# browserdotsys/vecchio

Hardware: NVIDIA B200
Metric: Mpaths/s (higher is better)
Workload: dtype f32

## Files before the change

vecchio_b200/csrc/vk_warpq.cu:

```cuda
#include "vk_warpq.cuh"

namespace VK_NS {

template <bool MEDIA, bool LEGACY, class W, int K, bool HYBRID, class D>
VKD void warpq_flat_body(const DScene& sc, const FlatProgram* flat, const DCamera& cam, const RenderArgs& a, const RenderBuffers& buf,
                         unsigned long long* unit_head, const D& dom) {
    extern __shared__ __align__(16) unsigned char vkq_raw[];
    const uint32_t lane = threadIdx.x & 31u, below = (1u << lane) - 1u;
    W& S = reinterpret_cast<W*>(vkq_raw)[threadIdx.x >> 5];
    const WqCtx<W> C = wq_ctx(dom, cam, a, S, unit_head, lane);
    uint32_t n_rays = 0, n_drop = 0, n_prims = 0;
    TraceCounters tc = {0u, 0u};
    constexpr uint32_t EXT_CAP = 32u * K;
    const uint32_t miss_cls = wq_black_miss(a) ? (uint32_t)VKQ_END : (uint32_t)VKQ_EMIT;
    wq_init(S, lane);
#pragma unroll 1
    for (;;) {
        uint32_t q, n_q, tail_q, head;
        wq_selfcheck(S, buf, lane, 0u);
        if (!wq_pick(S, wq_counts(S), EXT_CAP, q, n_q, tail_q)) break;
        const uint32_t n = wq_pop(S, q, n_q, tail_q, q == VKQ_EXT ? EXT_CAP : 32u, lane, head);
        if (q != VKQ_EXT) {
            wq_shade_batch<LEGACY, !HYBRID>(sc, C, dom, buf, q, n, head, n_drop);
            continue;
        }
        wq_converge();
        float3 o[K], d[K];
        float tm[K], best_t[K];
        bool live[K];
        uint32_t best_hit[K], slot[K];
        MediumXi xi[K];
#pragma unroll
        for (int k = 0; k < K; ++k) {
            const uint32_t e = lane + 32u * k;
            live[k] = e < n;
            slot[k] = S.ring[VKQ_EXT][(head + (live[k] ? e : 0u)) & W::RMASK];
            const float4 ro = S.ro[slot[k]], rd = S.rd[slot[k]];
            o[k] = f3(ro);
            d[k] = f3(rd);
            tm[k] = ro.w;
            xi[k].table = nullptr;
            xi[k].depth = __float_as_uint(rd.w);
            xi[k].rng.key = make_uint2(a.seed_lo, a.seed_hi);
            xi[k].rng.pixel = MEDIA ? S.px[slot[k]] : 0u;
            xi[k].rng.sample = MEDIA ? __float_as_uint(S.bt[slot[k]].w) : 0u;
            if (MEDIA) dom_slot_rng(dom, a, xi[k].rng);
        }
        TraceHit sub[K];
        trace_flat_k<K, MEDIA, HYBRID>(sc, *flat, o, d, tm, live, 0.001f, xi, best_t, best_hit, sub, &tc);
#pragma unroll
        for (int k = 0; k < K; ++k) {
            uint32_t cls = VKQ_NONE;
            if (live[k]) {
                ++n_rays;
                n_prims += flat->n;
                uint32_t prim = VK_REF_NONE, hi = 0u;
                cls = miss_cls;
                if (HYBRID && best_hit[k] == 0xFFFFFFFEu) {
                    prim = sub[k].prim;
                    hi = (sub[k].inst ? (0x80000000u | VKD_INDEX(sub[k].inst)) : 0u) | (sub[k].face << 28);
                    cls = wq_class_of(sc, prim, sub[k].inst);
                } else if (best_hit[k] != 0xFFFFFFFFu) {
                    cls = best_hit[k] >> 8;
                    best_hit[k] = VKF_HIT_INDEX(best_hit[k]);
                    prim = 1u;
                    if (HYBRID) {
                        const FlatHit& fh = flat->hits[best_hit[k]];
                        prim = fh.prim & ~VKD_DUP;
                        hi = (fh.inst ? (0x80000000u | VKD_INDEX(fh.inst)) : 0u) | (fh.face << 28);
                    }
                }
                S.hp[slot[k]] = make_uint4(__float_as_uint(best_t[k]), prim, hi, best_hit[k]);
            }
            if (k == 0 || n > 32u * k) wq_push(S, cls, slot[k], lane, below);
        }
    }
    wq_flush_counters(buf, lane, n_rays, n_drop, tc.nodes, n_prims + tc.prims);
}

#ifndef VKQ_BVH_IDLE
#define VKQ_BVH_IDLE 8u
#endif
#ifndef VKQ_NODE_STEPS
#define VKQ_NODE_STEPS 4
#endif
template <bool MEDIA, bool LEGACY, class W, class D>
VKD void warpq_bvh_body(const DScene& sc, const DCamera& cam, const RenderArgs& a, const RenderBuffers& buf, unsigned long long* unit_head,
                        const D& dom) {
    extern __shared__ __align__(16) unsigned char vkq_raw[];
    const uint32_t lane = threadIdx.x & 31u, below = (1u << lane) - 1u;
    W& S = reinterpret_cast<W*>(vkq_raw)[threadIdx.x >> 5];
    const WqCtx<W> C = wq_ctx(dom, cam, a, S, unit_head, lane);
    uint32_t n_rays = 0, n_drop = 0;
    TraceCounters tc = {0u, 0u};
    const uint32_t miss_cls = wq_black_miss(a) ? (uint32_t)VKQ_END : (uint32_t)VKQ_EMIT;
    wq_init(S, lane);

    Trav T;
    T.ref = VKD_DONE;
    T.sp = 0;
    T.enter = false;
    T.cur_inst = 0;
    T.co = T.cd = T.cinv = f3(0.0f, 0.0f, 0.0f);
    T.best.t = 0.0f;
    T.best.prim = VK_REF_NONE;
    T.best.inst = 0;
    T.best.face = 0;
    float3 o = f3(0.0f, 0.0f, 0.0f), d = o;
    float tm = 0.0f;
    uint32_t cur = 0xFFFFFFFFu;
    MediumXi xi;
    xi.table = nullptr;
    xi.depth = 0;
    xi.rng.key = make_uint2(a.seed_lo, a.seed_hi);
    xi.rng.pixel = 0;
    xi.rng.sample = 0;
#pragma unroll 1
    for (;;) {
        const bool done_lane = T.ref == VKD_DONE;
        const uint32_t m_done = __ballot_sync(0xFFFFFFFFu, done_lane);
        if ((uint32_t)__popc(m_done) >= VKQ_BVH_IDLE) {
            const bool fin = done_lane && cur != 0xFFFFFFFFu;
            if (__ballot_sync(0xFFFFFFFFu, fin) != 0u) {
                uint32_t cls = VKQ_NONE, slot = 0u;
                if (fin) {
                    slot = cur;
                    cur = 0xFFFFFFFFu;
                    S.hp[slot] = make_uint4(__float_as_uint(T.best.t), T.best.prim,
                                            (T.best.inst ? (0x80000000u | VKD_INDEX(T.best.inst)) : 0u) | (T.best.face << 28), 0u);
                    cls = T.best.prim == VK_REF_NONE ? miss_cls : wq_class_of(sc, T.best.prim, T.best.inst);
                }
                wq_push(S, cls, slot, lane, below);
            }
            wq_selfcheck(S, buf, lane, (uint32_t)__popc(__ballot_sync(0xFFFFFFFFu, cur != 0xFFFFFFFFu)));
            const WqCounts cnt = wq_counts(S);
            const uint32_t n_ext = __reduce_max_sync(0xFFFFFFFFu, cnt.c01.x);
            if (n_ext != 0u) {
                uint32_t head;
                const uint32_t take = wq_pop(S, VKQ_EXT, n_ext, cnt.c01.y, (uint32_t)__popc(m_done), lane, head);
                const uint32_t rank = (uint32_t)__popc(m_done & below);
                if (done_lane && rank < take) {
                    cur = S.ring[VKQ_EXT][(head + rank) & W::RMASK];
                    const float4 ro = S.ro[cur], rd = S.rd[cur];
                    o = f3(ro);
                    d = f3(rd);
                    tm = ro.w;
                    xi.depth = __float_as_uint(rd.w);
                    if (MEDIA) {
                        xi.rng.pixel = S.px[cur];
                        xi.rng.sample = __float_as_uint(S.bt[cur].w);
                        dom_slot_rng(dom, a, xi.rng);
                    }
                    trav_init(T, sc, o, d, CUDART_INF_F);
                    ++n_rays;
                }
            }
            const uint32_t m_act = __ballot_sync(0xFFFFFFFFu, T.ref != VKD_DONE);
            if (32u - (uint32_t)__popc(m_act) >= VKQ_BVH_IDLE) {
                uint32_t q, n_q, tail_q, head;
                if (wq_pick(S, wq_counts(S), 0u, q, n_q, tail_q)) {
                    const uint32_t n = wq_pop(S, q, n_q, tail_q, 32u, lane, head);
                    wq_shade_batch<LEGACY, false>(sc, C, dom, buf, q, n, head, n_drop);
                    continue;
                }
                if (m_act == 0u) break;
            }
        }
        wq_converge();
#pragma unroll 1
        for (int k = 0; k < VKQ_NODE_STEPS && trav_at_node(T); ++k) trav_node_step(T, sc, 0.001f, tc);
        if (T.ref != VKD_DONE && !trav_at_node(T)) trav_prim_step<MEDIA>(T, sc, o, d, tm, 0.001f, xi, tc);
    }
    wq_flush_counters(buf, lane, n_rays, n_drop, tc.nodes, tc.prims);
}

using WqFlat = WqWarp<VKQ_N_FLAT, VKQ_RN_FLAT>;
using WqMedia = WqWarp<VKQ_N_MEDIA, VKQ_RN_MEDIA>;
using WqBvh = WqWarp<VKQ_N_BVH, VKQ_RN_BVH>;
using WqHyb = WqWarp<VKQ_N_HYB, VKQ_RN_HYB>;
static_assert(VKQ_WARPS <= 15, "one named barrier per warp of the CTA");

template <bool MEDIA, bool LEGACY, class D>
__global__ void __launch_bounds__(32 * VKQ_WARPS, VKQ_MINB_BVH) k_warpq(const DScene sc, const DCamera cam, const RenderArgs a, const RenderBuffers buf,
                                                                    unsigned long long* unit_head, const __grid_constant__ D dom) {
    warpq_bvh_body<MEDIA, LEGACY, WqBvh>(sc, cam, a, buf, unit_head, dom);
}
template <bool LEGACY, class D>
__global__ void __launch_bounds__(32 * VKQ_WARPS, VKQ_MINB_FLAT) k_warpq_flat(const DScene sc, const __grid_constant__ FlatProgram flat, const DCamera cam,
                                                                          const RenderArgs a, const RenderBuffers buf, unsigned long long* unit_head,
                                                                          const __grid_constant__ D dom) {
    warpq_flat_body<false, LEGACY, WqFlat, VKQ_K_FLAT, false>(sc, &flat, cam, a, buf, unit_head, dom);
}
template <bool LEGACY, class D>
__global__ void __launch_bounds__(32 * VKQ_WARPS, VKQ_MINB_MEDIA) k_warpq_flat_media(const DScene sc, const __grid_constant__ FlatProgram flat,
                                                                                 const DCamera cam, const RenderArgs a, const RenderBuffers buf,
                                                                                 unsigned long long* unit_head, const __grid_constant__ D dom) {
    warpq_flat_body<true, LEGACY, WqMedia, VKQ_K_MEDIA, false>(sc, &flat, cam, a, buf, unit_head, dom);
}
#if !VK_SIMPLE
template <bool MEDIA, bool LEGACY, class D>
__global__ void __launch_bounds__(32 * VKQ_WARPS, VKQ_MINB_HYB) k_warpq_hybrid(const DScene sc, const __grid_constant__ FlatProgram flat, const DCamera cam,
                                                                            const RenderArgs a, const RenderBuffers buf, unsigned long long* unit_head,
                                                                            const __grid_constant__ D dom) {
    warpq_flat_body<MEDIA, LEGACY, WqHyb, 1, true>(sc, &flat, cam, a, buf, unit_head, dom);
}
#endif

template <class D>
cudaError_t launch_warpq(const DScene& sc, const FlatProgram* flat, const DCamera& cam, const RenderArgs& a, const RenderBuffers& b,
                         unsigned long long* unit_head, int sm_count, bool legacy, cudaStream_t st, const D& dom) {
    int bps = 0;
    cudaError_t e;
    const bool media = sc.has_media != 0u;
#define VKQ_LAUNCH_FLAT(KERNEL, WARP)                                                                                  \
    {                                                                                                                  \
        const size_t smem = VKQ_WARPS * sizeof(WARP);                                                                  \
        if ((e = warpq_prepare(KERNEL, smem, &bps)) != cudaSuccess) return e;                                          \
        KERNEL<<<sm_count * (bps < 1 ? 1 : bps), 32 * VKQ_WARPS, smem, st>>>(sc, *flat, cam, a, b, unit_head, dom);    \
    }
#define VKQ_LAUNCH_BVH(KERNEL)                                                                                         \
    {                                                                                                                  \
        const size_t smem = VKQ_WARPS * sizeof(WqBvh);                                                                 \
        if ((e = warpq_prepare(KERNEL, smem, &bps)) != cudaSuccess) return e;                                          \
        KERNEL<<<sm_count * (bps < 1 ? 1 : bps), 32 * VKQ_WARPS, smem, st>>>(sc, cam, a, b, unit_head, dom);           \
    }
#if VK_SIMPLE
    (void)legacy;
    if (media) VKQ_LAUNCH_FLAT((k_warpq_flat_media<false, D>), WqMedia) else VKQ_LAUNCH_FLAT((k_warpq_flat<false, D>), WqFlat)
#else
#define VKQ_LAUNCH_HYB(M, G) VKQ_LAUNCH_FLAT((k_warpq_hybrid<M, G, D>), WqHyb)
    if (flat && flat->n && flat->n_bvh) {
        if (media) { if (legacy) VKQ_LAUNCH_HYB(true, true) else VKQ_LAUNCH_HYB(true, false) }
        else { if (legacy) VKQ_LAUNCH_HYB(false, true) else VKQ_LAUNCH_HYB(false, false) }
    } else if (flat && flat->n) {
        if (media) { if (legacy) VKQ_LAUNCH_FLAT((k_warpq_flat_media<true, D>), WqMedia) else VKQ_LAUNCH_FLAT((k_warpq_flat_media<false, D>), WqMedia) }
        else { if (legacy) VKQ_LAUNCH_FLAT((k_warpq_flat<true, D>), WqFlat) else VKQ_LAUNCH_FLAT((k_warpq_flat<false, D>), WqFlat) }
    } else {
        if (media) { if (legacy) VKQ_LAUNCH_BVH((k_warpq<true, true, D>)) else VKQ_LAUNCH_BVH((k_warpq<true, false, D>)) }
        else { if (legacy) VKQ_LAUNCH_BVH((k_warpq<false, true, D>)) else VKQ_LAUNCH_BVH((k_warpq<false, false, D>)) }
    }
#undef VKQ_LAUNCH_HYB
#endif
#undef VKQ_LAUNCH_FLAT
#undef VKQ_LAUNCH_BVH
    return cudaGetLastError();
}
#define VKQ_INSTANTIATE(D)                                                                                             \
    template cudaError_t launch_warpq(const DScene&, const FlatProgram*, const DCamera&, const RenderArgs&, const RenderBuffers&, \
                                      unsigned long long*, int, bool, cudaStream_t, const D&);
VKQ_INSTANTIATE(OneFrame)
VKQ_INSTANTIATE(FrameArgs)
VKQ_INSTANTIATE(ListArgs)
VKQ_INSTANTIATE(FrameListArgs)
#undef VKQ_INSTANTIATE

}
```

vecchio_b200/csrc/vk_warpq.cuh:

```cuda
#pragma once
#include "vk_device.cuh"

namespace VK_NS {

#ifndef VKQ_WARPS
#define VKQ_WARPS 4
#endif
#ifndef VKQ_N_FLAT
#define VKQ_N_FLAT 176
#endif
#ifndef VKQ_RN_FLAT
#define VKQ_RN_FLAT 256
#endif
#ifndef VKQ_K_FLAT
#define VKQ_K_FLAT 2
#endif
#ifndef VKQ_MINB_FLAT
#define VKQ_MINB_FLAT 4
#endif
#ifndef VKQ_N_MEDIA
#define VKQ_N_MEDIA 144
#endif
#ifndef VKQ_RN_MEDIA
#define VKQ_RN_MEDIA 256
#endif
#ifndef VKQ_K_MEDIA
#define VKQ_K_MEDIA 1
#endif
#ifndef VKQ_MINB_MEDIA
#define VKQ_MINB_MEDIA 5
#endif
#ifndef VKQ_N_BVH
#define VKQ_N_BVH 120
#endif
#ifndef VKQ_RN_BVH
#define VKQ_RN_BVH 128
#endif
#ifndef VKQ_MINB_BVH
#define VKQ_MINB_BVH 6
#endif
#ifndef VKQ_N_HYB
#define VKQ_N_HYB 120
#endif
#ifndef VKQ_RN_HYB
#define VKQ_RN_HYB 128
#endif
#ifndef VKQ_MINB_HYB
#define VKQ_MINB_HYB 6
#endif
#ifndef VKQ_REGEN_MIN
#define VKQ_REGEN_MIN 32u
#endif
#define VKQ_CHUNK 256u
enum { VKQ_EXT = 0, VKQ_END = 1, VKQ_EMIT = 2, VKQ_DIEL = 3, VKQ_METAL = 4, VKQ_DIFF = 5, VKQ_DIFFI = 6, VKQ_NQ = 7,
       VKQ_SPH = 7, VKQ_BOX = 8, VKQ_LEAF = 9, VKQ_NQ_STEP = 10, VKQ_NONE = 15 };
static_assert(VKF_HITC(0, 0, 0) >> 8 == VKQ_EMIT && VKF_HITC(0, 1, 0) >> 8 == VKQ_DIEL && VKF_HITC(0, 2, 0) >> 8 == VKQ_METAL &&
              VKF_HITC(0, 3, 0) >> 8 == VKQ_DIFF && VKF_HITC(0, 3, 1) >> 8 == VKQ_DIFFI, "the flat program's class-tagged ids name these queues");

template <int N_, int RN_>
struct WqWarp {
    static constexpr uint32_t N = N_, RMASK = RN_ - 1, NQ = VKQ_NQ;
    static_assert((RN_ & (RN_ - 1)) == 0 && RN_ >= N_ && RN_ <= 256, "ring capacity: power of two, >= slots, byte indices");
    float4 ro[N_];
    float4 rd[N_];
    float4 bt[N_];
    uint4 hp[N_];
    uint32_t px[N_];
    uint8_t ring[VKQ_NQ][RN_];
    uint2 ct[8];
    uint32_t cur_s, cur_y, cur_x, left;
    uint32_t exhausted;
    VKD void mark_new(uint32_t) {}
};


#ifndef VKQ_CONVERGE
#define VKQ_CONVERGE 1
#endif
VKD void wq_converge() {
#if VKQ_CONVERGE
    asm volatile("barrier.sync.aligned %0, 32;" ::"r"((threadIdx.x >> 5) + 1u) : "memory");
#endif
}
template <class W>
struct WqCtx {
    const DCamera& cam;
    const RenderArgs& a;
    W& S;
    uint32_t chunks_per_row, chunks_per_sample;
    unsigned long long n_chunks;
    unsigned long long* unit_head;
    uint32_t lane, below;
};

template <class D> VKD uint32_t wq_row_length(const D&, const RenderArgs& a) { return a.width; }
VKD uint32_t wq_row_length(const ListArgs& ls, const RenderArgs&) { return ls.n; }
VKD uint32_t wq_row_length(const FrameListArgs& fl, const RenderArgs&) { return fl.ls.n; }
template <class D> VKD uint32_t wq_rows(const D&, const RenderArgs& a) { return a.height; }
VKD uint32_t wq_rows(const ListArgs&, const RenderArgs&) { return 1u; }
VKD uint32_t wq_rows(const FrameListArgs&, const RenderArgs&) { return 1u; }
template <class W, class D>
VKD WqCtx<W> wq_ctx(const D& dom, const DCamera& cam, const RenderArgs& a, W& S, unsigned long long* unit_head, uint32_t lane) {
    const uint32_t cpr = (wq_row_length(dom, a) + VKQ_CHUNK - 1u) / VKQ_CHUNK, cps = cpr * wq_rows(dom, a);
    return WqCtx<W>{cam, a, S, cpr, cps, (unsigned long long)cps * a.spp_count * dom_frames(dom), unit_head, lane, (1u << lane) - 1u};
}
template <class W>
VKD void wq_chunk(const WqCtx<W>& C, const OneFrame&, unsigned long long c) {
    W& S = C.S;
    const uint32_t sb = (uint32_t)(c / C.chunks_per_sample);
    const uint32_t r = (uint32_t)(c - (unsigned long long)sb * C.chunks_per_sample);
    const uint32_t row = r / C.chunks_per_row, x0 = (r - row * C.chunks_per_row) * VKQ_CHUNK;
    S.left = min(VKQ_CHUNK, C.a.width - x0);
    S.cur_s = sb;
    S.cur_y = row;
    S.cur_x = x0;
}
template <class W>
VKD void wq_chunk(const WqCtx<W>& C, const FrameArgs&, unsigned long long c) {
    W& S = C.S;
    const unsigned long long fs = c / C.chunks_per_sample;
    const uint32_t f = (uint32_t)(fs / C.a.spp_count);
    const uint32_t r = (uint32_t)(c - fs * C.chunks_per_sample);
    const uint32_t row = r / C.chunks_per_row, x0 = (r - row * C.chunks_per_row) * VKQ_CHUNK;
    S.left = min(VKQ_CHUNK, C.a.width - x0);
    S.cur_s = (uint32_t)(fs - (unsigned long long)f * C.a.spp_count);
    S.cur_y = f * C.a.height + row;
    S.cur_x = x0;
}
template <class W>
VKD void wq_chunk(const WqCtx<W>& C, const ListArgs& ls, unsigned long long c) {
    W& S = C.S;
    const uint32_t sb = (uint32_t)(c / C.chunks_per_sample);
    const uint32_t x0 = ((uint32_t)c - sb * C.chunks_per_sample) * VKQ_CHUNK;
    S.left = min(VKQ_CHUNK, ls.n - x0);
    S.cur_s = sb;
    S.cur_y = 0u;
    S.cur_x = x0;
}
template <class W>
VKD void wq_chunk(const WqCtx<W>& C, const FrameListArgs& fl, unsigned long long c) { wq_chunk(C, fl.ls, c); }
template <class W>
VKD uint32_t wq_camera_ray(const WqCtx<W>& C, const OneFrame&, uint32_t x, uint32_t y, PathRng& rng, float3& o, float3& d, float& time) {
    camera_get_ray(C.cam, rng, x, y, C.a.width, C.a.height, o, d, time);
    return rng.pixel;
}
template <class W>
VKD uint32_t wq_camera_ray(const WqCtx<W>& C, const FrameArgs& fr, uint32_t x, uint32_t y, PathRng& rng, float3& o, float3& d, float& time) {
    const uint32_t p = rng.pixel;
    const uint32_t f = y / C.a.height;
    y -= f * C.a.height;
    rng.pixel = y * C.a.width + x;
    rng.key = frame_key(C.a, f);
    camera_get_ray(fr.cams[f], rng, x, y, C.a.width, C.a.height, o, d, time);
    return p;
}
template <class W>
VKD uint32_t wq_camera_ray(const WqCtx<W>& C, const ListArgs& ls, uint32_t x, uint32_t y, PathRng& rng, float3& o, float3& d, float& time) {
    rng.pixel = ls.list[x];
    y = rng.pixel / C.a.width;
    x = rng.pixel - y * C.a.width;
    camera_get_ray(C.cam, rng, x, y, C.a.width, C.a.height, o, d, time);
    return rng.pixel;
}
template <class W>
VKD uint32_t wq_camera_ray(const WqCtx<W>& C, const FrameListArgs& fl, uint32_t x, uint32_t, PathRng& rng, float3& o, float3& d, float& time) {
    const uint32_t g = fl.ls.list[x];
    rng.pixel = g;
    const uint32_t f = dom_unit_frame(fl, C.a, rng);
    const uint32_t y = rng.pixel / C.a.width;
    camera_get_ray(fl.fr.cams[f], rng, rng.pixel - y * C.a.width, y, C.a.width, C.a.height, o, d, time);
    return g;
}

template <class W>
VKD void wq_push(W& S, uint32_t cls, uint32_t slot, uint32_t lane, uint32_t below) {
    const uint32_t m = __match_any_sync(0xFFFFFFFFu, cls);
    const uint32_t leader = __ffs(m) - 1u;
    uint32_t pos = 0;
    if (lane == leader && cls != VKQ_NONE) {
        const uint2 c = S.ct[cls];
        pos = c.y;
        S.ct[cls] = make_uint2(c.x + (uint32_t)__popc(m), c.y + (uint32_t)__popc(m));
    }
    pos = __shfl_sync(0xFFFFFFFFu, pos, leader);
    if (cls != VKQ_NONE) S.ring[cls][(pos + __popc(m & below)) & W::RMASK] = (uint8_t)slot;
    __syncwarp();
}

template <class W, class D>
VKD bool wq_regen(const WqCtx<W>& C, const D& dom, bool want, uint32_t slot) {
    W& S = C.S;
    const uint32_t m = __ballot_sync(0xFFFFFFFFu, want);
    if (m == 0u) return false;
    const uint32_t need = (uint32_t)__popc(m), rank = (uint32_t)__popc(m & C.below);
    uint32_t served = 0, s = 0, y = 0, x = 0;
    bool got = false;
#pragma unroll 1
    while (served < need) {
        uint32_t left = __reduce_max_sync(0xFFFFFFFFu, S.left);
        if (left == 0u) {
            if (__any_sync(0xFFFFFFFFu, S.exhausted != 0u)) break;
            __syncwarp();
            if (C.lane == 0) {
                const unsigned long long c = atomicAdd(C.unit_head, 1ull);
                if (c >= C.n_chunks) S.exhausted = 1u;
                else wq_chunk(C, dom, c);
            }
            __syncwarp();
            if (__any_sync(0xFFFFFFFFu, S.exhausted != 0u)) break;
            left = __reduce_max_sync(0xFFFFFFFFu, S.left);
        }
        const uint32_t take = min(need - served, left);
        const uint32_t cs = S.cur_s, cy = S.cur_y, cx = S.cur_x;
        if (want && rank >= served && rank < served + take) {
            x = cx + (rank - served);
            y = cy;
            s = cs;
            got = true;
        }
        __syncwarp();
        if (C.lane == 0) {
            S.cur_x = cx + take;
            S.left = left - take;
        }
        __syncwarp();
        served += take;
    }
    if (got) {
        PathRng rng;
        rng.pixel = y * C.a.width + x;
        rng.sample = C.a.spp_begin + s;
        rng.key = make_uint2(C.a.seed_lo, C.a.seed_hi);
        float3 o, d;
        float time;
        const uint32_t p = wq_camera_ray(C, dom, x, y, rng, o, d, time);
        S.ro[slot] = make_float4(o.x, o.y, o.z, time);
        S.rd[slot] = make_float4(d.x, d.y, d.z, __uint_as_float(1u));
        S.bt[slot] = make_float4(1.0f, 1.0f, 1.0f, __uint_as_float(rng.sample));
        S.px[slot] = p;
        S.mark_new(slot);
    }
    return got;
}

VKD bool wq_black_miss(const RenderArgs& a) {
    return !(a.flags & VK_FLAG_SKY_BACKGROUND) && a.background.x == 0.0f && a.background.y == 0.0f && a.background.z == 0.0f;
}
VKD uint32_t wq_class_of(const DScene& sc, uint32_t prim, uint32_t inst) {
    uint32_t mat;
    const uint32_t i = VKD_INDEX(prim);
    switch (VKD_TYPE(prim)) {
    case VK_T_SPHERE: mat = __ldg(&sc.sphere_mat[i]); break;
    case VK_T_MSPHERE: mat = __float_as_uint(__ldg(&sc.mspheres[3 * i + 2]).y); break;
    case VK_T_RECT: mat = __float_as_uint(__ldg(&sc.rects[2 * i + 1]).z); break;
    case VK_T_BOX: mat = __float_as_uint(__ldg(&sc.boxes[2 * i]).w); break;
    default: mat = __float_as_uint(__ldg(&sc.media[i]).z); break;
    }
    const uint32_t t = __ldg(&sc.materials[mat]).x;
    return t == VK_M_DIFFUSE_LIGHT ? VKQ_EMIT : t == VK_M_DIELECTRIC ? VKQ_DIEL : t == VK_M_METAL ? VKQ_METAL : (inst ? VKQ_DIFFI : VKQ_DIFF);
}

struct WqCounts {
    uint4 c01, c23, c45, c67;
};
template <class W>
VKD WqCounts wq_counts(const W& S) {
    WqCounts c;
    c.c01 = *reinterpret_cast<const uint4*>(&S.ct[0]);
    c.c23 = *reinterpret_cast<const uint4*>(&S.ct[2]);
    c.c45 = *reinterpret_cast<const uint4*>(&S.ct[4]);
    c.c67 = *reinterpret_cast<const uint4*>(&S.ct[6]);
    return c;
}
template <class W>
VKD bool wq_pick(const W& S, const WqCounts& c, uint32_t ext_cap, uint32_t& q, uint32_t& n_q, uint32_t& tail_q) {
    const uint32_t w = (ext_cap ? ext_cap : 32u) * 8u;
    uint32_t key = ext_cap ? c.c01.x * 256u + VKQ_EXT : 0u;
    key = max(key, c.c23.x * w + VKQ_EMIT);
    key = max(key, c.c45.z * w + VKQ_DIFF);
    key = max(key, c.c67.x * w + VKQ_DIFFI);
    key = max(key, c.c23.z * w + VKQ_DIEL);
    key = max(key, c.c45.x * w + VKQ_METAL);
    key = max(key, c.c01.z * w + VKQ_END);
    key = __reduce_max_sync(0xFFFFFFFFu, key);
    q = key & 7u;
    const uint2 e = S.ct[q];
    n_q = e.x;
    tail_q = e.y;
    return (key >> 3) != 0u;
}
template <class W>
VKD uint32_t wq_pop(W& S, uint32_t q, uint32_t n_q, uint32_t tail_q, uint32_t cap, uint32_t lane, uint32_t& head) {
    const uint32_t n = min(n_q, cap);
    head = tail_q - n_q;
    __syncwarp();
    if (lane == 0) S.ct[q].x = n_q - n;
    __syncwarp();
    return n;
}

#ifndef VKQ_FAST_RESOLVE
#define VKQ_FAST_RESOLVE 1
#endif
template <bool LEGACY, bool FLAT, class W, class D>
VKD void wq_shade_batch(const DScene& sc, const WqCtx<W>& C, const D& dom, const RenderBuffers& buf, uint32_t q, uint32_t n, uint32_t head, uint32_t& n_drop) {
    W& S = C.S;
    const RenderArgs& a = C.a;
    const uint32_t lane = C.lane;
    const bool act = lane < n;
    const uint32_t slot = S.ring[q][(head + (act ? lane : 0u)) & W::RMASK];
    bool alive = false, ended = false;
    if (q != VKQ_END) {
        if (act) {
            const float4 ro = S.ro[slot], rd = S.rd[slot], bt = S.bt[slot];
            const uint4 hp = S.hp[slot];
            float3 o = f3(ro), d = f3(rd), beta = f3(bt), L = f3(0.0f, 0.0f, 0.0f);
            float time = ro.w;
            uint32_t depth = __float_as_uint(rd.w);
            const uint32_t pixel = S.px[slot], prim = hp.y;
            bool valid = true;
            if (prim == VK_REF_NONE) {
                L = beta * miss_color(a, d);
            } else {
                PathRng rng;
                rng.pixel = pixel;
                rng.sample = __float_as_uint(bt.w);
                rng.key = make_uint2(a.seed_lo, a.seed_hi);
                dom_slot_rng(dom, a, rng);
                HitRecD rec;
                bool direct = false;
                uint32_t leaf = prim, hi = hp.z;
                if (FLAT) {
                    const float4 fs1 = __ldg(&sc.flat_shade[2u * hp.w + 1u]);
                    leaf = __float_as_uint(fs1.y);
                    hi = __float_as_uint(fs1.z);
#if VKQ_FAST_RESOLVE && !VK_STRICT
                    const float4 fs = __ldg(&sc.flat_shade[2u * hp.w]);
                    const uint32_t fl = __float_as_uint(fs.w);
                    if (fl & 1u) {
                        direct = true;
                        const float3 nw = f3(fs);
                        const bool toward = dot3(d, nw) < 0.0f;
                        rec.t = __uint_as_float(hp.x);
                        rec.p = at(o, d, rec.t);
                        rec.normal = toward ? nw : -nw;
                        rec.front = (toward ? 1u : 0u) ^ ((fl >> 1) & 1u);
                        rec.u = 0.0f;
                        rec.v = 0.0f;
                        rec.mat = __float_as_uint(fs1.x);
                        rec.m = __ldg(&sc.materials[rec.mat]);
                    }
#endif
                }
                if (!direct) {
                    TraceHit h;
                    h.t = __uint_as_float(hp.x);
                    h.prim = leaf;
                    h.inst = (hi & 0x80000000u) ? (((uint32_t)VK_T_XFORM << 28) | (hi & 0x07FFFFFFu)) : 0u;
                    h.face = (hi >> 28) & 7u;
                    resolve_hit(sc, h, o, d, time, false, rec);
                }
                alive = LEGACY ? shade_legacy(sc, rec, rng, depth, o, d, time, beta, L, valid)
                               : shade(sc, rec, rng, depth, o, d, time, beta, L, valid);
                if (alive && ++depth > a.max_depth) alive = false;
                if (alive && !(finite3(d) && finite3(o))) {
                    valid = false;
                    alive = false;
                }
            }
            if (alive) {
                S.ro[slot] = make_float4(o.x, o.y, o.z, time);
                S.rd[slot] = make_float4(d.x, d.y, d.z, __uint_as_float(depth));
                S.bt[slot] = make_float4(beta.x, beta.y, beta.z, bt.w);
                S.mark_new(slot);
            } else {
                if (valid && finite3(L)) dom_accumulate(dom, buf, pixel, L);
                else ++n_drop;
                ended = true;
            }
        }
    } else {
        ended = act;
    }
    const uint32_t m_end = __ballot_sync(0xFFFFFFFFu, ended);
    bool to_end = false;
    if (q == VKQ_END || (uint32_t)__popc(m_end) >= VKQ_REGEN_MIN) alive = wq_regen(C, dom, ended, slot) || alive;
    else to_end = ended;
    const uint32_t m_ext = __ballot_sync(0xFFFFFFFFu, alive), m_q = __ballot_sync(0xFFFFFFFFu, to_end);
    const uint2 c_ext = S.ct[VKQ_EXT], c_end = S.ct[VKQ_END];
    if (alive) S.ring[VKQ_EXT][(c_ext.y + __popc(m_ext & C.below)) & W::RMASK] = (uint8_t)slot;
    if (to_end) S.ring[VKQ_END][(c_end.y + __popc(m_q & C.below)) & W::RMASK] = (uint8_t)slot;
    __syncwarp();
    if (lane == 0) {
        S.ct[VKQ_EXT] = make_uint2(c_ext.x + (uint32_t)__popc(m_ext), c_ext.y + (uint32_t)__popc(m_ext));
        if (m_q) S.ct[VKQ_END] = make_uint2(c_end.x + (uint32_t)__popc(m_q), c_end.y + (uint32_t)__popc(m_q));
    }
    __syncwarp();
}

#ifndef VKQ_SELFCHECK
#define VKQ_SELFCHECK 0
#endif
template <class W>
VKD void wq_selfcheck(const W& S, const RenderBuffers& buf, uint32_t lane, uint32_t in_flight) {
#if VKQ_SELFCHECK
    uint32_t seen[8] = {0, 0, 0, 0, 0, 0, 0, 0};
    uint32_t bad = 0, total = 0;
    for (uint32_t q = 0; q < W::NQ; ++q) {
        const uint2 c = S.ct[q];
        total += c.x;
        if (c.x > W::N) ++bad;
        for (uint32_t i0 = 0; i0 < c.x; i0 += 32u) {
            const uint32_t i = i0 + lane;
            const bool have = i < c.x;
            const uint32_t slot = have ? S.ring[q][(c.y - c.x + i) & W::RMASK] : 0u;
            if (have && slot >= W::N) ++bad;
            const uint32_t same = __match_any_sync(0xFFFFFFFFu, have ? slot : 0x10000u + lane);
            if (have && __popc(same) != 1) ++bad;
#pragma unroll
            for (uint32_t w = 0; w < 8; ++w) {
                const uint32_t mine = (have && (slot >> 5) == w) ? (1u << (slot & 31u)) : 0u;
                const uint32_t all = __reduce_or_sync(0xFFFFFFFFu, mine);
                if (mine & seen[w]) ++bad;
                seen[w] |= all;
            }
        }
    }
    if (total + in_flight > W::N) ++bad;
    if (bad) atomicAdd(&buf.counters[5], (unsigned long long)bad);
#else
    (void)S, (void)buf, (void)lane, (void)in_flight;
#endif
}

template <class W>
VKD void wq_init(W& S, uint32_t lane) {
    if (lane < W::NQ + (W::NQ & 1u)) S.ct[lane] = make_uint2(0u, 0u);
    for (uint32_t i = lane; i < W::N; i += 32u) S.ring[VKQ_END][i] = (uint8_t)i;
    if (lane == 0) {
        S.left = 0u;
        S.exhausted = 0u;
        S.cur_s = 0u;
        S.cur_y = 0u;
        S.cur_x = 0u;
    }
    __syncwarp();
    if (lane == 0) S.ct[VKQ_END] = make_uint2(W::N, W::N);
    __syncwarp();
}
VKD void wq_flush_counters(const RenderBuffers& buf, uint32_t lane, uint32_t n_rays, uint32_t n_drop, uint32_t n_nodes, uint32_t n_prims) {
    unsigned long long w_rays = n_rays, w_drop = n_drop, w_nodes = n_nodes, w_prims = n_prims;
#pragma unroll
    for (int off = 16; off > 0; off >>= 1) {
        w_rays += __shfl_xor_sync(0xFFFFFFFFu, w_rays, off);
        w_drop += __shfl_xor_sync(0xFFFFFFFFu, w_drop, off);
        w_nodes += __shfl_xor_sync(0xFFFFFFFFu, w_nodes, off);
        w_prims += __shfl_xor_sync(0xFFFFFFFFu, w_prims, off);
    }
    if (lane == 0) {
        atomicAdd(&buf.counters[3], w_nodes);
        atomicAdd(&buf.counters[4], w_prims);
        atomicAdd(&buf.counters[0], w_rays);
        if (w_drop) atomicAdd(&buf.counters[1], w_drop);
    }
}


#ifndef VKQ_CAP_BPS
#define VKQ_CAP_BPS 0
#endif
template <class K> static cudaError_t warpq_prepare(K kernel, size_t smem, int* blocks_per_sm) {
    cudaError_t e = cudaFuncSetAttribute(kernel, cudaFuncAttributeMaxDynamicSharedMemorySize, (int)smem);
    if (e != cudaSuccess) return e;
    e = cudaOccupancyMaxActiveBlocksPerMultiprocessor(blocks_per_sm, kernel, 32 * VKQ_WARPS, smem);
    if (e != cudaSuccess) return e;
    if (VKQ_CAP_BPS && *blocks_per_sm > VKQ_CAP_BPS) *blocks_per_sm = VKQ_CAP_BPS;
    const size_t need = (size_t)(*blocks_per_sm < 1 ? 1 : *blocks_per_sm) * (smem + 1024);
    int pct = (int)((need * 100 + 233472 - 1) / 233472);
    pct = pct > 100 ? 100 : pct;
    e = cudaFuncSetAttribute(kernel, cudaFuncAttributePreferredSharedMemoryCarveout, pct);
    if (e != cudaSuccess) return e;
    e = cudaOccupancyMaxActiveBlocksPerMultiprocessor(blocks_per_sm, kernel, 32 * VKQ_WARPS, smem);
    if (VKQ_CAP_BPS && *blocks_per_sm > VKQ_CAP_BPS) *blocks_per_sm = VKQ_CAP_BPS;
    return e;
}

}
```

Baseline: 11570.

## Split diffuse queue by mixture coin and reclassify direct-resolvable diffuse hits

Adds an optional mode, off by default, that draws the bounce random numbers at trace time and uses the mixture coin to split diffuse hits into a separate cosine-lobe queue. Each shading batch then takes a single lobe branch, which is meant to cut warp divergence. It also adds a default-on DIRECT_DIFF path that moves hits flagged as directly resolvable from the DIFFI queue to the DIFF queue. The cost is an extra global load per hit and more template variants. The split mode adds one ring queue and shifts RNG work into the trace stage.

```diff
diff --git a/vecchio_b200/csrc/vk_warpq.cu b/vecchio_b200/csrc/vk_warpq.cu
--- a/vecchio_b200/csrc/vk_warpq.cu
+++ b/vecchio_b200/csrc/vk_warpq.cu
@@ -12,6 +12,9 @@
     uint32_t n_rays = 0, n_drop = 0, n_prims = 0;
     TraceCounters tc = {0u, 0u};
     constexpr uint32_t EXT_CAP = 32u * K;
+    constexpr bool SPLIT = wq_mix_split<LEGACY>() && !HYBRID;
+    constexpr bool DIRECT_DIFF = wq_direct_diff<LEGACY>() && !HYBRID;
+    static_assert(W::NQ == (SPLIT ? VKQ_NQ_SPLIT : VKQ_NQ), "the cosine-lobe queue exists exactly when the coin is split");
     const uint32_t miss_cls = wq_black_miss(a) ? (uint32_t)VKQ_END : (uint32_t)VKQ_EMIT;
     wq_init(S, lane);
 #pragma unroll 1
@@ -21,7 +24,7 @@
         if (!wq_pick(S, wq_counts(S), EXT_CAP, q, n_q, tail_q)) break;
         const uint32_t n = wq_pop(S, q, n_q, tail_q, q == VKQ_EXT ? EXT_CAP : 32u, lane, head);
         if (q != VKQ_EXT) {
-            wq_shade_batch<LEGACY, !HYBRID>(sc, C, dom, buf, q, n, head, n_drop);
+            wq_shade_batch<LEGACY, !HYBRID, SPLIT>(sc, C, dom, buf, q, n, head, n_drop);
             continue;
         }
         wq_converge();
@@ -48,6 +51,19 @@
         }
         TraceHit sub[K];
         trace_flat_k<K, MEDIA, HYBRID>(sc, *flat, o, d, tm, live, 0.001f, xi, best_t, best_hit, sub, &tc);
+        uint4 xb[K];
+#pragma unroll
+        for (int k = 0; k < K; ++k) {
+            if (SPLIT) {
+                PathRng rng = xi[k].rng;
+                if (!MEDIA) {
+                    rng.pixel = S.px[slot[k]];
+                    rng.sample = __float_as_uint(S.bt[slot[k]].w);
+                    dom_slot_rng(dom, a, rng);
+                }
+                xb[k] = rng.block(xi[k].depth, 0u);
+            }
+        }
 #pragma unroll
         for (int k = 0; k < K; ++k) {
             uint32_t cls = VKQ_NONE;
@@ -70,7 +86,15 @@
                         hi = (fh.inst ? (0x80000000u | VKD_INDEX(fh.inst)) : 0u) | (fh.face << 28);
                     }
                 }
-                S.hp[slot[k]] = make_uint4(__float_as_uint(best_t[k]), prim, hi, best_hit[k]);
+                if (DIRECT_DIFF && cls == VKQ_DIFFI && (__float_as_uint(__ldg(&sc.flat_shade[2u * best_hit[k]]).w) & 1u)) cls = VKQ_DIFF;
+                uint32_t t_bits = __float_as_uint(best_t[k]);
+                if (SPLIT) {
+                    if (cls == VKQ_DIFF && !(u01(xb[k].x) < 0.5f)) cls = VKQ_DIFFC;
+                    prim = cls == VKQ_DIEL ? xb[k].x : xb[k].y;
+                    hi = xb[k].z;
+                    t_bits |= xb[k].x & 0x80000000u;
+                }
+                S.hp[slot[k]] = make_uint4(t_bits, prim, hi, best_hit[k]);
             }
             if (k == 0 || n > 32u * k) wq_push(S, cls, slot[k], lane, below);
         }
@@ -174,8 +198,8 @@
     wq_flush_counters(buf, lane, n_rays, n_drop, tc.nodes, tc.prims);
 }
 
-using WqFlat = WqWarp<VKQ_N_FLAT, VKQ_RN_FLAT>;
-using WqMedia = WqWarp<VKQ_N_MEDIA, VKQ_RN_MEDIA>;
+template <bool LEGACY> using WqFlat = WqWarp<VKQ_N_FLAT, VKQ_RN_FLAT, wq_mix_split<LEGACY>() ? VKQ_NQ_SPLIT : VKQ_NQ>;
+template <bool LEGACY> using WqMedia = WqWarp<VKQ_N_MEDIA, VKQ_RN_MEDIA, wq_mix_split<LEGACY>() ? VKQ_NQ_SPLIT : VKQ_NQ>;
 using WqBvh = WqWarp<VKQ_N_BVH, VKQ_RN_BVH>;
 using WqHyb = WqWarp<VKQ_N_HYB, VKQ_RN_HYB>;
 static_assert(VKQ_WARPS <= 15, "one named barrier per warp of the CTA");
@@ -189,13 +213,13 @@
 __global__ void __launch_bounds__(32 * VKQ_WARPS, VKQ_MINB_FLAT) k_warpq_flat(const DScene sc, const __grid_constant__ FlatProgram flat, const DCamera cam,
                                                                           const RenderArgs a, const RenderBuffers buf, unsigned long long* unit_head,
                                                                           const __grid_constant__ D dom) {
-    warpq_flat_body<false, LEGACY, WqFlat, VKQ_K_FLAT, false>(sc, &flat, cam, a, buf, unit_head, dom);
+    warpq_flat_body<false, LEGACY, WqFlat<LEGACY>, VKQ_K_FLAT, false>(sc, &flat, cam, a, buf, unit_head, dom);
 }
 template <bool LEGACY, class D>
 __global__ void __launch_bounds__(32 * VKQ_WARPS, VKQ_MINB_MEDIA) k_warpq_flat_media(const DScene sc, const __grid_constant__ FlatProgram flat,
                                                                                  const DCamera cam, const RenderArgs a, const RenderBuffers buf,
                                                                                  unsigned long long* unit_head, const __grid_constant__ D dom) {
-    warpq_flat_body<true, LEGACY, WqMedia, VKQ_K_MEDIA, false>(sc, &flat, cam, a, buf, unit_head, dom);
+    warpq_flat_body<true, LEGACY, WqMedia<LEGACY>, VKQ_K_MEDIA, false>(sc, &flat, cam, a, buf, unit_head, dom);
 }
 #if !VK_SIMPLE
 template <bool MEDIA, bool LEGACY, class D>
@@ -226,15 +250,15 @@
     }
 #if VK_SIMPLE
     (void)legacy;
-    if (media) VKQ_LAUNCH_FLAT((k_warpq_flat_media<false, D>), WqMedia) else VKQ_LAUNCH_FLAT((k_warpq_flat<false, D>), WqFlat)
+    if (media) VKQ_LAUNCH_FLAT((k_warpq_flat_media<false, D>), WqMedia<false>) else VKQ_LAUNCH_FLAT((k_warpq_flat<false, D>), WqFlat<false>)
 #else
 #define VKQ_LAUNCH_HYB(M, G) VKQ_LAUNCH_FLAT((k_warpq_hybrid<M, G, D>), WqHyb)
     if (flat && flat->n && flat->n_bvh) {
         if (media) { if (legacy) VKQ_LAUNCH_HYB(true, true) else VKQ_LAUNCH_HYB(true, false) }
         else { if (legacy) VKQ_LAUNCH_HYB(false, true) else VKQ_LAUNCH_HYB(false, false) }
     } else if (flat && flat->n) {
-        if (media) { if (legacy) VKQ_LAUNCH_FLAT((k_warpq_flat_media<true, D>), WqMedia) else VKQ_LAUNCH_FLAT((k_warpq_flat_media<false, D>), WqMedia) }
-        else { if (legacy) VKQ_LAUNCH_FLAT((k_warpq_flat<true, D>), WqFlat) else VKQ_LAUNCH_FLAT((k_warpq_flat<false, D>), WqFlat) }
+        if (media) { if (legacy) VKQ_LAUNCH_FLAT((k_warpq_flat_media<true, D>), WqMedia<true>) else VKQ_LAUNCH_FLAT((k_warpq_flat_media<false, D>), WqMedia<false>) }
+        else { if (legacy) VKQ_LAUNCH_FLAT((k_warpq_flat<true, D>), WqFlat<true>) else VKQ_LAUNCH_FLAT((k_warpq_flat<false, D>), WqFlat<false>) }
     } else {
         if (media) { if (legacy) VKQ_LAUNCH_BVH((k_warpq<true, true, D>)) else VKQ_LAUNCH_BVH((k_warpq<true, false, D>)) }
         else { if (legacy) VKQ_LAUNCH_BVH((k_warpq<false, true, D>)) else VKQ_LAUNCH_BVH((k_warpq<false, false, D>)) }
diff --git a/vecchio_b200/csrc/vk_warpq.cuh b/vecchio_b200/csrc/vk_warpq.cuh
--- a/vecchio_b200/csrc/vk_warpq.cuh
+++ b/vecchio_b200/csrc/vk_warpq.cuh
@@ -52,21 +52,26 @@
 #define VKQ_REGEN_MIN 32u
 #endif
 #define VKQ_CHUNK 256u
+#ifndef VKQ_MIX_SPLIT
+#define VKQ_MIX_SPLIT 0
+#endif
+template <bool LEGACY> constexpr bool wq_mix_split() { return VKQ_MIX_SPLIT && (VK_SIMPLE || VK_LIGHT0) && !LEGACY; }
 enum { VKQ_EXT = 0, VKQ_END = 1, VKQ_EMIT = 2, VKQ_DIEL = 3, VKQ_METAL = 4, VKQ_DIFF = 5, VKQ_DIFFI = 6, VKQ_NQ = 7,
-       VKQ_SPH = 7, VKQ_BOX = 8, VKQ_LEAF = 9, VKQ_NQ_STEP = 10, VKQ_NONE = 15 };
+       VKQ_DIFFC = 7, VKQ_NQ_SPLIT = 8, VKQ_SPH = 7, VKQ_BOX = 8, VKQ_LEAF = 9, VKQ_NQ_STEP = 10, VKQ_NONE = 15 };
 static_assert(VKF_HITC(0, 0, 0) >> 8 == VKQ_EMIT && VKF_HITC(0, 1, 0) >> 8 == VKQ_DIEL && VKF_HITC(0, 2, 0) >> 8 == VKQ_METAL &&
               VKF_HITC(0, 3, 0) >> 8 == VKQ_DIFF && VKF_HITC(0, 3, 1) >> 8 == VKQ_DIFFI, "the flat program's class-tagged ids name these queues");
 
-template <int N_, int RN_>
+template <int N_, int RN_, int NQ_ = VKQ_NQ>
 struct WqWarp {
-    static constexpr uint32_t N = N_, RMASK = RN_ - 1, NQ = VKQ_NQ;
+    static constexpr uint32_t N = N_, RMASK = RN_ - 1, NQ = NQ_;
     static_assert((RN_ & (RN_ - 1)) == 0 && RN_ >= N_ && RN_ <= 256, "ring capacity: power of two, >= slots, byte indices");
+    static_assert(NQ_ == VKQ_NQ || NQ_ == VKQ_NQ_SPLIT, "the flat kernels' queues, with or without the cosine-lobe queue");
     float4 ro[N_];
     float4 rd[N_];
     float4 bt[N_];
     uint4 hp[N_];
     uint32_t px[N_];
-    uint8_t ring[VKQ_NQ][RN_];
+    uint8_t ring[NQ_][RN_];
     uint2 ct[8];
     uint32_t cur_s, cur_y, cur_x, left;
     uint32_t exhausted;
@@ -279,6 +284,7 @@
     key = max(key, c.c23.x * w + VKQ_EMIT);
     key = max(key, c.c45.z * w + VKQ_DIFF);
     key = max(key, c.c67.x * w + VKQ_DIFFI);
+    if (W::NQ == VKQ_NQ_SPLIT) key = max(key, c.c67.z * w + VKQ_DIFFC);
     key = max(key, c.c23.z * w + VKQ_DIEL);
     key = max(key, c.c45.x * w + VKQ_METAL);
     key = max(key, c.c01.z * w + VKQ_END);
@@ -302,8 +308,15 @@
 #ifndef VKQ_FAST_RESOLVE
 #define VKQ_FAST_RESOLVE 1
 #endif
-template <bool LEGACY, bool FLAT, class W, class D>
+#ifndef VKQ_DIRECT_DIFF
+#define VKQ_DIRECT_DIFF 1
+#endif
+template <bool LEGACY> constexpr bool wq_direct_diff() {
+    return (VKQ_DIRECT_DIFF || VKQ_MIX_SPLIT) && VKQ_FAST_RESOLVE && !VK_STRICT && (VK_SIMPLE || VK_LIGHT0) && !LEGACY;
+}
+template <bool LEGACY, bool FLAT, bool SPLIT = false, class W, class D>
 VKD void wq_shade_batch(const DScene& sc, const WqCtx<W>& C, const D& dom, const RenderBuffers& buf, uint32_t q, uint32_t n, uint32_t head, uint32_t& n_drop) {
+    static_assert(!SPLIT || (FLAT && !LEGACY), "the stored words are the flat program's HEAD-integrator bounce");
     W& S = C.S;
     const RenderArgs& a = C.a;
     const uint32_t lane = C.lane;
@@ -319,7 +332,7 @@
             uint32_t depth = __float_as_uint(rd.w);
             const uint32_t pixel = S.px[slot], prim = hp.y;
             bool valid = true;
-            if (prim == VK_REF_NONE) {
+            if (SPLIT ? hp.w == 0xFFFFFFFFu : prim == VK_REF_NONE) {
                 L = beta * miss_color(a, d);
             } else {
                 PathRng rng;
@@ -341,7 +354,7 @@
                         direct = true;
                         const float3 nw = f3(fs);
                         const bool toward = dot3(d, nw) < 0.0f;
-                        rec.t = __uint_as_float(hp.x);
+                        rec.t = SPLIT ? fabsf(__uint_as_float(hp.x)) : __uint_as_float(hp.x);
                         rec.p = at(o, d, rec.t);
                         rec.normal = toward ? nw : -nw;
                         rec.front = (toward ? 1u : 0u) ^ ((fl >> 1) & 1u);
@@ -354,14 +367,21 @@
                 }
                 if (!direct) {
                     TraceHit h;
-                    h.t = __uint_as_float(hp.x);
+                    h.t = SPLIT ? fabsf(__uint_as_float(hp.x)) : __uint_as_float(hp.x);
                     h.prim = leaf;
                     h.inst = (hi & 0x80000000u) ? (((uint32_t)VK_T_XFORM << 28) | (hi & 0x07FFFFFFu)) : 0u;
                     h.face = (hi >> 28) & 7u;
                     resolve_hit(sc, h, o, d, time, false, rec);
                 }
-                alive = LEGACY ? shade_legacy(sc, rec, rng, depth, o, d, time, beta, L, valid)
-                               : shade(sc, rec, rng, depth, o, d, time, beta, L, valid);
+                if (SPLIT) {
+                    const uint32_t coin = q == VKQ_DIFFC ? 0x80000000u : q == VKQ_DIFFI ? (hp.x & 0x80000000u) : 0u;
+                    BounceXiTable xt = {make_uint4(q == VKQ_DIEL ? hp.y : coin, hp.y, hp.z, 0u), 0u};
+                    if (!VK_SIMPLE && q == VKQ_METAL) xt.r = rng.block(depth, 0u);
+                    alive = shade_xi(sc, rec, xt, o, d, time, beta, L, valid);
+                } else {
+                    alive = LEGACY ? shade_legacy(sc, rec, rng, depth, o, d, time, beta, L, valid)
+                                   : shade(sc, rec, rng, depth, o, d, time, beta, L, valid);
+                }
                 if (alive && ++depth > a.max_depth) alive = false;
                 if (alive && !(finite3(d) && finite3(o))) {
                     valid = false;
```

New measurement: 11130, median of 6. -3.8%, worse.
